# WesleyHsieh0806/TAO-Amodal

Measured on AMD Instinct MI355X. Metric: box-pair IoU+match throughput, higher is better.
Workload: dtype f64

## Files before the change

include/tao_amodal_hip.h:

```cpp
#ifndef TAO_AMODAL_HIP_H
#define TAO_AMODAL_HIP_H

#include <stddef.h>
#include <stdint.h>

#ifdef __cplusplus
extern "C" {
#endif

#define TAOAMD_N_THR 10
#define TAOAMD_N_REC 101
#define TAOAMD_LVIS_RNG 6
#define TAOAMD_TAO_RNG 20

#define TAOAMD_GT_IGNORE 1
#define TAOAMD_GT_OOF 2
#define TAOAMD_GT_ID_HIDDEN 4
#define TAOAMD_DT_IGNORE_UNMATCHED 1
#define TAOAMD_DT_NO_CONSUME 2

#define TAOAMD_OK 0
#define TAOAMD_ERR_HIP 1
#define TAOAMD_ERR_ARG 2
#define TAOAMD_ERR_TOO_LARGE 3
// ... 117 lines not shown
                                  const int64_t *b, int64_t *out, int64_t *n_out);

int taoamd_track_iou_plan_host(int64_t n_cells, const int32_t *cell_dt_off_host,
                               const int32_t *cell_gt_off_host,
                               const int64_t *cell_iou_off_host,
                               const int32_t *trk_meta_host, int64_t *sizes,
                               int32_t *tasks_host, int32_t *task_rows_host,
                               int32_t *task_pairs_host, int64_t *task_out_host);
int taoamd_track_iou_plan_spans_host(int64_t n_cells, const int32_t *cell_dt_off_host,
                                     const int32_t *cell_gt_off_host,
                                     const int64_t *cell_iou_off_host,
                                     const int32_t *trk_meta_host, int64_t *sizes,
                                     int32_t *tasks_host, int32_t *task_rows_host,
                                     int32_t *task_pairs_host, int64_t *task_out_host,
                                     int64_t *zero_out_host);

#define TAOAMD_MAX_GT_PER_CELL 3072
int taoamd_match(int64_t n_cells, const int32_t *cell_dt_off,
                 const int32_t *cell_gt_off, const int64_t *cell_iou_off,
                 int32_t max_gt_per_cell, const double *dt_box,
                 const double *gt_box, const double *iou, int32_t n_rng,
                 const uint32_t *gt_rng, const uint32_t *dt_rng,
                 const uint8_t *gt_flags, const uint8_t *dt_flags,
                 const int32_t *dst, int64_t out_stride, uint64_t *matched,
                 uint64_t *ignored, int32_t *match_gt, double *ious_out,
                 const int32_t *dt_group, const uint32_t *dt_meta,
                 const int32_t *groups, int32_t n_groups, const int32_t *singles,
                 int32_t n_singles, void *stream);

int taoamd_match_compact(int64_t n_cells, const int32_t *cell_dt_off,
                         const int32_t *cell_gt_off, int32_t max_gt_per_cell,
                         const double *dt_box, const double *gt_box, int32_t n_rng,
                         const uint32_t *gt_rng, const uint8_t *gt_flags,
                         const uint8_t *dt_flags, uint64_t *rows, uint32_t *compact,
                         const int32_t *dt_group, const uint32_t *dt_meta,
                         const int32_t *groups, int32_t n_groups, const int32_t *singles,
                         int32_t n_singles, void *stream);
int taoamd_expand_rows(int64_t n_dt, int32_t n_rng, const uint32_t *compact,
                       uint64_t *rows, void *stream);

int taoamd_flat_map(int64_t n, const int64_t *image_id, const int64_t *category_id,
                    const double *bbox, const double *area_in, int64_t n_img,
                    const int64_t *img_ids, int64_t n_cat, const int64_t *cat_ids,
                    int32_t *img, int32_t *cat, double *area, int32_t *img_count,
                    int32_t *img_start, int32_t *img_first, int32_t *status,
                    void *stream);
int taoamd_flat_rank_drop(int64_t n, const int32_t *order, const int32_t *img,
                          const int32_t *img_start, int32_t max_dets,
                          uint8_t *dropped, void *stream);
int taoamd_flat_filter(int64_t n, const int32_t *unit, const int32_t *cat,
                       const double *area, const int64_t *category_id,
                       const uint8_t *dropped, int32_t n_unit, int64_t n_gkeys,
                       const int32_t *gkeys, const int32_t *unit_row,
                       const int64_t *neg_off, const int64_t *neg_val,
                       const int64_t *nel_off, const int64_t *nel_val,
                       int32_t area_flag, int32_t *key, uint8_t *flags,
                       int32_t *n_keep, void *stream);
int taoamd_flat_gather(int64_t n_keep, const int32_t *order, const double *score,
                       const uint8_t *flags, const int32_t *key,
                       const double *bbox, int32_t n_unit, int32_t *dt_row,
                       double *dt_score, uint8_t *dt_flags, int32_t *dt_key,
                       int32_t *dt_cat, double *dt_box, void *stream);
int taoamd_flat_count_bad(int64_t n, const double *bbox, const uint8_t *dropped,
                          int32_t *count, void *stream);
int taoamd_flat_ordscore(int64_t n, const int32_t *img, const int32_t *img_count,
                         const double *score, int32_t max_dets, double *out,
                         void *stream);
int taoamd_flat_ordinal(int64_t n, const int32_t *order, const int32_t *img,
                        const int32_t *img_start, int32_t max_dets,
                        int32_t *ordinal, uint8_t *dropped, void *stream);
int taoamd_flat_merge_cat(int64_t n, const int64_t *category_id, int64_t n_merge,
                          const int64_t *merge_src, const int64_t *merge_dst,
                          int64_t n_cat, const int64_t *cat_ids, int64_t *merged_id,
                          int32_t *cat, void *stream);
int taoamd_flat_split64(int64_t n, const int64_t *key, const int32_t *order,
                        int32_t *lo, int32_t *hi, void *stream);
int taoamd_flat_compose(int64_t n, const int32_t *outer, const int32_t *inner,
                        int32_t *out, void *stream);
int taoamd_flat_gather_cols(int64_t n, const int32_t *idx, const int32_t *src_i32,
                            int32_t *out_i32, const double *src_f64,
                            double *out_f64, const uint8_t *src_u8,
                            uint8_t *out_u8, void *stream);
int taoamd_flat_track_of(int64_t n, const int32_t *order, const int32_t *run_id,
                         const int32_t *run_start, const int64_t *video_id,
                         int32_t *trk, int32_t *status, void *stream);
int taoamd_flat_keys(int64_t n, const int32_t *img, const int32_t *ordinal,
                     const uint8_t *dropped, const int32_t *cat, const double *area,
                     const int32_t *trk, const int32_t *img_rank,
                     const int32_t *visit_rank, const double *img_frame,
                     const int32_t *tl_pos, double M, double *keep_key,
                     double *visit_key, double *frame_key, double *pos_key,
                     int32_t *trk_keep, int32_t *trk_sel, void *stream);
int taoamd_flat_track_kept(int64_t n_runs, const int32_t *run_trk,
                           const int32_t *run_start, int64_t n_sorted,
                           const int32_t *order_k, const double *score,
                           const int64_t *merged_id, double *trk_score,
                           int32_t *trk_first_kept, int32_t *status, void *stream);
int taoamd_flat_track_sel(int64_t n_runs, const int32_t *run_trk,
                          const int32_t *run_start, int64_t n_sorted,
                          const int32_t *order_s, const double *area,
                          const double *visit_key, const int32_t *img,
                          double *sel_area, int32_t *sel_len, int32_t *sel_frames,
                          double *sel_first, void *stream);
int taoamd_flat_track_filter(int64_t n_runs, const int32_t *run_trk,
                             const int32_t *sel_len, const int32_t *trk_first_kept,
                             const int32_t *cat, const int64_t *merged_id,
                             const int64_t *video_id, const int64_t *track_id,
                             int64_t n_vid, const int64_t *vid_ids, int64_t n_gkeys,
                             const int32_t *gkeys, const int32_t *vid_row,
                             const int64_t *neg_off, const int64_t *neg_val,
                             const int64_t *nel_off, const int64_t *nel_val,
                             int32_t *key, uint8_t *flags, int32_t *n_keep,
                             int32_t *status, void *stream);
int taoamd_flat_frames(int64_t n_trk, const int32_t *trk_run,
                       const int32_t *run_start, int64_t n_runs, int64_t n_sorted,
                       const int32_t *order_s, const int32_t *img,
                       const int32_t *tl_pos, const double *bbox,
                       const int32_t *frame_off, int32_t *frame_pos,
                       double *frame_box, void *stream);
int taoamd_flat_scan(int64_t n, const int32_t *count, int32_t *start,
                     int32_t *status2, void *stream);
size_t taoamd_flat_runs_workspace(int64_t n);
int taoamd_flat_runs(int64_t n, const int32_t *sorted_key, int32_t *run_id,
                     int32_t *run_key, int32_t *run_start, int32_t *n_runs,
                     void *workspace, size_t workspace_bytes, void *stream);
int taoamd_flat_runs_by(int64_t n, const int32_t *key, const int32_t *order,
                        int32_t *run_id, int32_t *run_key, int32_t *run_start,
                        int32_t *n_runs, void *workspace, size_t workspace_bytes,
                        void *stream);
int taoamd_flat_runs64_by(int64_t n, const int64_t *key, const int32_t *order,
                          int32_t *run_id, int64_t *run_key, int32_t *run_start,
                          int32_t *n_runs, void *workspace, size_t workspace_bytes,
                          void *stream);
int taoamd_flat_remap(int64_t n, const int32_t *id, const int32_t *map,
                      int32_t *out, void *stream);

int taoamd_match_plan_host(int64_t n_cells, const int32_t *cell_dt_off_host,
                           const int32_t *cell_gt_off_host, int32_t cap_d,
                           int32_t cap_g, int32_t cap_cell_g, int64_t *sizes,
                           int32_t *groups_host, int32_t *singles_host);

size_t taoamd_sort_workspace(int64_t n);
int taoamd_sort_by_cat_score(int64_t n, const int32_t *dt_cat,
                             const double *dt_score, int32_t *order,
                             int32_t *dst, void *workspace,
                             size_t workspace_bytes, void *stream);

#define TAOAMD_SORT_CHUNK (16 * 2816)
int taoamd_sort_plan_host(int32_t n_cat, const int32_t *cat_off_host, int64_t *sizes,
                          int32_t *chunks, int32_t *split_list, int32_t *stile_chunk,
                          int32_t *bucket_chunk);
size_t taoamd_sort_sampled_workspace(int64_t n, int64_t n_buckets, int32_t merge);
int taoamd_sort_sampled_cap_limit(int32_t limit);
int taoamd_sort_sampled(int64_t n, int32_t n_cat, const int32_t *cat_off,
                        const int32_t *tile_off, int32_t n_tiles, int32_t max_segment,
                        const double *dt_score, int32_t n_chunks, const int32_t *chunks,
                        int32_t n_split, const int32_t *split_list, int32_t n_stiles,
                        const int32_t *stile_chunk, int32_t n_buckets,
                        const int32_t *bucket_chunk, int32_t *order, int32_t *dst,
                        void *workspace, size_t workspace_bytes, void *stream);

#define TAOAMD_SEGMENT_TILE 2816
size_t taoamd_sort_segments_workspace(int64_t n);
int taoamd_sort_segments(int64_t n, int32_t n_cat, const int32_t *cat_off,
                         const int32_t *tile_off, int32_t n_tiles,
                         int32_t max_segment, const int32_t *dt_cat,
                         const double *dt_score, int32_t *order, int32_t *dst,
                         void *workspace, size_t workspace_bytes, void *stream);

int taoamd_gather_rows(int64_t n, int32_t n_words, const uint64_t *src_matched,
                       const uint64_t *src_ignored, int64_t src_stride,
                       const int32_t *order, uint64_t *dst_matched,
                       uint64_t *dst_ignored, void *stream);

size_t taoamd_accumulate_workspace(int64_t n_dt, int32_t n_cat, int32_t n_rng);
size_t taoamd_compact_elems(int32_t n_cat, int32_t n_rng);
int taoamd_accumulate_compact(int64_t n_dt, int32_t n_cat, int32_t n_rng,
                              const int32_t *cat_off, const uint64_t *matched,
                              const uint64_t *ignored, const int32_t *num_gt,
                              int32_t k_begin, int32_t k_end, int32_t max_segment,
                              double *val, double *rec, void *workspace,
                              size_t workspace_bytes, void *stream);
int taoamd_finalize(int32_t n_cat, int32_t n_rng, const int32_t *num_gt,
                    const double *val, const double *rec, double *precision,
                    double *recall, void *stream);
int taoamd_accumulate(int64_t n_dt, int32_t n_cat, int32_t n_rng,
                      const int32_t *cat_off, const uint64_t *matched,
                      const uint64_t *ignored,
                      const int32_t *num_gt, int32_t max_segment, double *precision,
                      double *recall, void *workspace, size_t workspace_bytes,
                      void *stream);
int taoamd_accumulate_error(const void *workspace, void *stream, int32_t *flag_host);
int taoamd_accumulate_chunked(int64_t n_dt, int32_t n_cat, int32_t n_rng,
                      const int32_t *cat_off, const uint64_t *matched,
                      const uint64_t *ignored,
                      const int32_t *num_gt, int32_t max_segment, double *precision,
                      double *recall, void *workspace, size_t workspace_bytes,
                      void *stream);
int taoamd_accumulate_compact_chunked(int64_t n_dt, int32_t n_cat, int32_t n_rng,
                              const int32_t *cat_off, const uint64_t *matched,
                              const uint64_t *ignored, const int32_t *num_gt,
                              int32_t k_begin, int32_t k_end, int32_t max_segment,
                              double *val, double *rec, void *workspace,
                              size_t workspace_bytes, void *stream);
int taoamd_accumulate_sweep_mode(int32_t mode);
int taoamd_accumulate_plan_kind(int64_t n_dt, int32_t n_rng, int32_t max_segment);
int taoamd_accumulate_spin_limit(int32_t polls);
int taoamd_accumulate_giveup_counter(uint32_t *device_word);
int taoamd_accumulate_prepare(int64_t n_dt, int32_t n_cat, int32_t n_rng,
                              const int32_t *cat_off, int32_t max_segment,
                              void *workspace, size_t workspace_bytes, void *stream);
int taoamd_accumulate_prepared(int64_t n_dt, int32_t n_cat, int32_t n_rng,
                      const int32_t *cat_off, const uint64_t *matched,
                      const uint64_t *ignored,
                      const int32_t *num_gt, int32_t max_segment, double *precision,
                      double *recall, void *workspace, size_t workspace_bytes,
                      void *stream);
int taoamd_accumulate_by_order(int64_t n_dt, int32_t n_cat, int32_t n_rng,
                               const int32_t *cat_off, const int32_t *order,
                               const uint64_t *matched, const uint64_t *ignored,
                               const int32_t *num_gt, int32_t max_segment,
                               double *precision, double *recall, void *workspace,
                               size_t workspace_bytes, void *stream);
int taoamd_accumulate_by_order_prepared(int64_t n_dt, int32_t n_cat, int32_t n_rng,
                               const int32_t *cat_off, const int32_t *order,
                               const uint64_t *matched, const uint64_t *ignored,
                               const int32_t *num_gt, int32_t max_segment,
                               double *precision, double *recall, void *workspace,
                               size_t workspace_bytes, void *stream);
int taoamd_accumulate_by_order_chunked(int64_t n_dt, int32_t n_cat, int32_t n_rng,
                               const int32_t *cat_off, const int32_t *order,
                               const uint64_t *matched, const uint64_t *ignored,
                               const int32_t *num_gt, int32_t max_segment,
                               double *precision, double *recall, void *workspace,
                               size_t workspace_bytes, void *stream);
int taoamd_accumulate_by_order_compact(int64_t n_dt, int32_t n_cat, int32_t n_rng,
                               const int32_t *cat_off, const int32_t *order,
                               const uint32_t *compact, const uint64_t *rows,
                               const int32_t *num_gt, int32_t max_segment,
                               double *precision, double *recall, void *workspace,
                               size_t workspace_bytes, int32_t prepared, void *stream);

size_t taoamd_score_at_recall_workspace(int64_t n_dt, int32_t n_cat, int32_t n_rng);
int taoamd_score_at_recall(int64_t n_dt, int32_t n_cat, int32_t n_rng,
                           const int32_t *cat_off, const int32_t *order,
                           const uint64_t *matched, const uint64_t *ignored,
                           const double *score, const int32_t *score_order,
                           const int32_t *num_gt, double *scores, void *workspace, size_t workspace_bytes,
                           void *stream);

#define TAOAMD_ERROR_TYPES_TILE 256
#define TAOAMD_ERROR_TYPES_MAX_RNG 8
size_t taoamd_error_types_workspace(int64_t n_dt, int64_t n_gt, int32_t n_rng);
int taoamd_error_types(int64_t n_dt, int64_t n_gt, int32_t n_img, int32_t n_cat,
                       int32_t n_rng, int32_t slot, double bg_thr,
                       const int32_t *dt_cat, const double *dt_box,
                       const uint8_t *dt_flags, const int32_t *dt_gt0,
                       const int32_t *match_gt, int64_t match_stride,
                       const int32_t *gt_cat, const double *gt_box,
                       const uint32_t *gt_rng, const int32_t *img_gt_off,
                       const int32_t *img_gt, const int32_t *img_dt_off,
                       const int32_t *img_dt, int64_t *dt_counts, int64_t *gt_counts,
                       uint8_t *dt_type, void *workspace, size_t workspace_bytes,
                       void *stream);

int taoamd_error_types_links(int64_t n_dt, int64_t n_gt, int32_t n_img, int32_t n_cat,
                             int32_t n_rng, int32_t slot, double bg_thr,
                             const int32_t *dt_cat, const double *dt_box,
                             const uint8_t *dt_flags, const int32_t *dt_gt0,
                             const int32_t *match_gt, int64_t match_stride,
                             const int32_t *gt_cat, const double *gt_box,
                             const uint32_t *gt_rng, const int32_t *img_gt_off,
                             const int32_t *img_gt, const int32_t *img_dt_off,
                             const int32_t *img_dt, int64_t *dt_counts, int64_t *gt_counts,
                             uint8_t *dt_type, int32_t *link_same, int32_t *link_other,
                             uint8_t *held, void *workspace, size_t workspace_bytes,
                             void *stream);

#define TAOAMD_ERROR_IMPACT_FIXES 9
#define TAOAMD_ERROR_IMPACT_CHUNK 256
size_t taoamd_error_impact_workspace(int64_t n_dt, int64_t n_gt, int32_t n_cat, int32_t n_rng);
int taoamd_error_impact(int64_t n_dt, int64_t n_gt, int32_t n_cat, int32_t n_rng,
                        const int32_t *cat_off, const int32_t *order, const double *score,
                        const int32_t *dt_cat, const uint8_t *dt_type,
                        const int32_t *link_same, const int32_t *link_other,
                        const int32_t *gt_cat, const uint32_t *gt_rng, const uint8_t *held,
                        double *precision, int32_t *num_gt, void *workspace,
                        size_t workspace_bytes, void *stream);

size_t taoamd_track_error_impact_workspace(int64_t n_dt, int64_t n_gt, int32_t n_cat,
                                           int32_t n_rng);
int taoamd_track_error_impact(int64_t n_dt, int64_t n_gt, int32_t n_cat, int32_t n_rng,
                              const int32_t *cat_off, const int32_t *order,
                              const double *score, const int32_t *dt_cat,
                              const uint8_t *dt_type, const int32_t *link_same,
                              const int32_t *link_other, const int32_t *gt_cat,
                              const uint32_t *gt_rng, const uint8_t *held, double *precision,
                              int32_t *num_gt, void *workspace, size_t workspace_bytes,
                              void *stream);

#define TAOAMD_CONFUSION_TILE 2048
size_t taoamd_confusion_workspace(int64_t n_dt, int64_t n_gt, int32_t n_cat, int32_t n_rng);
int taoamd_confusion_count(int64_t n_dt, int64_t n_gt, int32_t n_cat, int32_t n_rng,
                           const int32_t *cat_off, const double *score, const int32_t *dt_cat,
                           const uint8_t *dt_type, const int32_t *link_other,
                           const int32_t *gt_cat, const uint8_t *held, int64_t *ent_off,
// ... 232 lines not shown
```

tao_amodal_amd/csrc/sort.hip:

```cpp
#include <algorithm>
#include <cstdlib>
#include <cstring>

#include "common.hpp"
#include "workspace.hpp"

using namespace taoamd;

#define RS_THREADS 256
#define RS_WAVES (RS_THREADS / WAVE)
#define RS_ITEMS 8
#define RS_TILE (RS_THREADS * RS_ITEMS)
#define RS_BINS 256
#define RS_PASSES 12

struct SortBufs {
    uint64_t *key[2];
    int32_t *idx[2];
    const int32_t *cat;
    uint32_t *block_hist;
    uint32_t *digit_total;
    int32_t *skip;
    int32_t *sel;
    int64_t n;
// ... 677 lines not shown
            L.key[i] = kin[src_of(i)];
            L.pos[i] = (uint16_t)i;
        }
    });
    const int32_t out = X.out_base;
#pragma nounroll
    for (int i = threadIdx.x; i < total; i += SEG_THREADS) {
        const int32_t p = out + seg_final_slot(L, i, total, repaired);
        const int32_t d = iin[src_of((int)(L.pos[i] & 0x0fffu))];
        if (a.order) a.order[p] = d;
        if (a.dst) a.dst[d] = p;
    }
}

#define MP_PER 11

template <class KA, class KB>
__device__ __forceinline__ int32_t merge_split(KA A, int32_t na, KB B, int32_t nb, int32_t o)
{
    int32_t lo = max(0, o - nb), hi = min(o, na);
    while (lo < hi) {
        const int32_t mid = (lo + hi) >> 1;
        if (A[mid] <= B[o - mid - 1]) lo = mid + 1; else hi = mid;
    }
    return lo;
}

__global__ __launch_bounds__(256) void seg_mpass_kernel(SegArgs a, int pass, int last,
                                                        int32_t longer_than)
{
    __shared__ uint64_t m_key[SEG_TILE];
    __shared__ int32_t m_idx[SEG_TILE];
    __shared__ int32_t m_split[2];
    static_assert(256 * MP_PER == SEG_TILE, "one workgroup = one tile-sized slice");
    int32_t lo = 0, hi = a.n_cat;
    while (hi - lo > 1) {
        const int32_t mid = (lo + hi) >> 1;
        if (a.tile_off[mid] <= (int32_t)blockIdx.x) lo = mid; else hi = mid;
    }
    const int32_t k = lo;
    const int32_t sb = a.cat_off[k], se = a.cat_off[k + 1];
    if (se - sb <= longer_than) return;
    const int32_t tb = sb + ((int32_t)blockIdx.x - a.tile_off[k]) * SEG_TILE;
    const int32_t len = min(SEG_TILE, se - tb);
    if (len <= 0) return;
    const int s = pass & 1;
    const uint64_t *__restrict__ kin = a.key[s];
    const int32_t *__restrict__ iin = a.idx[s];
    const int64_t L = (int64_t)SEG_TILE << pass;
    const int64_t base = sb + ((tb - sb) / (2 * L)) * (2 * L);
    const int32_t a0 = (int32_t)base, a1 = (int32_t)min(base + L, (int64_t)se);
    const int32_t b1 = (int32_t)min((int64_t)a1 + L, (int64_t)se);
    const int32_t na = a1 - a0, nb = b1 - a1;
    const int32_t o0 = tb - a0;
    auto emit = [&](int32_t p, uint64_t kx, int32_t ix) {
        if (last) {
            if (a.order) a.order[p] = ix;
            if (a.dst) a.dst[ix] = p;
        } else {
            a.key[s ^ 1][p] = kx;
            a.idx[s ^ 1][p] = ix;
        }
    };
    if (nb <= 0) {
        for (int32_t i = threadIdx.x; i < len; i += 256) emit(tb + i, kin[tb + i], iin[tb + i]);
        return;
    }
    if (threadIdx.x == 0) m_split[0] = merge_split(kin + a0, na, kin + a1, nb, o0);
    if (threadIdx.x == 64) m_split[1] = merge_split(kin + a0, na, kin + a1, nb, o0 + len);
    __syncthreads();
    const int32_t i0 = m_split[0], i1 = m_split[1];
    const int32_t j0 = o0 - i0;
    const int32_t pa = i1 - i0, pb = len - pa;
    for (int32_t i = threadIdx.x; i < len; i += 256) {
        const int32_t src = i < pa ? a0 + i0 + i : a1 + j0 + (i - pa);
        m_key[i] = kin[src];
        m_idx[i] = iin[src];
    }
    __syncthreads();
    const int32_t q0 = min(len, (int32_t)threadIdx.x * MP_PER);
    const int32_t q1 = min(len, q0 + MP_PER);
    if (q0 >= q1) return;
    const uint64_t *A = m_key, *B = m_key + pa;
    int32_t ia = merge_split(A, pa, B, pb, q0);
    int32_t ib = q0 - ia;
    for (int32_t q = q0; q < q1; q++) {
        const bool takeA = ib >= pb || (ia < pa && A[ia] <= B[ib]);
        const int32_t from = takeA ? ia : pa + ib;
        emit(tb + q, m_key[from], m_idx[from]);
        ia += takeA ? 1 : 0;
        ib += takeA ? 0 : 1;
    }
}

static void seg_layout(Carve &c, int64_t n, SegArgs &a)
{
    if (n < 1) n = 1;
    key_idx_layout(c, n, a);
    a.bnd = c.take<int32_t>(((size_t)n / SEG_TILE + 2) * SEG_BND_PER_SLOT);
}

extern "C" size_t taoamd_sort_segments_workspace(int64_t n)
{
    SegArgs a;
    return measure([&](Carve &c) { seg_layout(c, n, a); });
}

extern "C" int taoamd_sort_segments(int64_t n, int32_t n_cat,
                                    const int32_t *cat_off,
                                    const int32_t *tile_off, int32_t n_tiles,
                                    int32_t max_segment, const int32_t *dt_cat,
                                    const double *dt_score, int32_t *order,
                                    int32_t *dst, void *workspace,
                                    size_t workspace_bytes, void *stream)
{
    if (n == 0 || n_cat == 0 || n_tiles == 0) return TAOAMD_OK;
    if (n > 0x7fffffff) return TAOAMD_ERR_TOO_LARGE;
    if (!cat_off || !tile_off || !dt_cat || !dt_score || !workspace) return TAOAMD_ERR_ARG;
    Carve c(workspace);
    SegArgs a;
    seg_layout(c, n, a);
    if (!c.fits(workspace, workspace_bytes)) return TAOAMD_ERR_WORKSPACE;
    hipStream_t s = (hipStream_t)stream;
    a.cat_off = cat_off; a.tile_off = tile_off; a.cat = dt_cat; a.score = dt_score;
    a.order = order; a.dst = dst; a.n = n; a.n_cat = n_cat; a.n_tiles = n_tiles;
    TAO_TIMED("seg_tile_kernel", s, seg_tile_kernel<<<(unsigned)n_tiles, SEG_THREADS, 0, s>>>(a));
    if (max_segment > SEG_TILE && max_segment <= (int64_t)SEG_KMERGE_TILES * SEG_TILE) {
        TAO_TIMED("seg_kmerge_kernel", s, seg_kmerge_kernel<<<(unsigned)((n + 255) / 256), 256, 0, s>>>(a));
    } else if (max_segment > SEG_TILE) {
        TAO_TIMED("seg_split_kernel", s, seg_split_kernel<<<(unsigned)n_cat, SEG_THREADS, 0, s>>>(a));
        TAO_TIMED("seg_bucket_kernel", s, seg_bucket_kernel<<<2u * (unsigned)n_tiles, SEG_THREADS, 0, s>>>(a));
        const int32_t longer_than = SEG_SPLIT_TILES * SEG_TILE;
        if (max_segment > longer_than) {
            int passes = 0;
            for (int64_t L = SEG_TILE; L < max_segment; L <<= 1) passes++;
            for (int p = 0; p < passes; p++)
                TAO_TIMED("seg_mpass_kernel", s, seg_mpass_kernel<<<(unsigned)n_tiles, 256, 0, s>>>(a, p, p == passes - 1, longer_than));
        }
    }
    TAO_LAUNCH_CHECK();
    return TAOAMD_OK;
}

#define SS_CAP 1024
#define SS_FAST 512
#define SS_TARGET 352
#define SS_CHUNK_TILES 16
#define SS_FIRST_MERGE_PASS 4
#define SS_OVER 32
#define SS_DIRECT 1024
#define SS_CHUNK (SS_CHUNK_TILES * SEG_TILE)
#define SS_MAXB 128
#define SS_HALF_CHUNK (SS_CHUNK / 2)

struct SsChunk {
    int32_t begin, n;
    int32_t bucket0, n_buckets;
    int32_t stile0;
    int32_t final;
    int32_t cat, pad;
};

struct SsArgs {
    const double *score;
    const SsChunk *chunks;
    const int32_t *split_list, *stile_chunk, *bucket_chunk;
    int32_t *cursor;
    uint64_t *spl_key;
    int32_t *spl_idx;
    uint64_t *slot_key;
    int32_t *slot_idx;
    uint64_t *key_out;
    int32_t *idx_out;
    int32_t *order, *dst;
    int32_t *redo;
    int32_t n_buckets, n_stiles, cap_limit;
};

static int g_ss_cap_limit = SS_CAP;

__host__ __device__ inline int ss_over(int32_t n) { return n > SS_HALF_CHUNK ? SS_OVER / 2 : SS_OVER; }

__device__ __forceinline__ uint32_t ss_mix(uint32_t x)
{
    x ^= x >> 16; x *= 0x7feb352du; x ^= x >> 15; x *= 0x846ca68bu; x ^= x >> 16;
    return x;
}

__device__ __forceinline__ uint64_t ss_shfl_xor64(uint64_t v, int j)
{
    const uint32_t lo = (uint32_t)__shfl_xor((int)(uint32_t)v, j, WAVE);
    const uint32_t hi = (uint32_t)__shfl_xor((int)(uint32_t)(v >> 32), j, WAVE);
    return ((uint64_t)hi << 32) | lo;
}

__device__ __forceinline__ double ss_fmin(double a, double b)
{
    double r;
    asm("v_min_f64 %0, %1, %2" : "=v"(r) : "v"(a), "v"(b));
    return r;
}
__device__ __forceinline__ double ss_fmax(double a, double b)
{
    double r;
    asm("v_max_f64 %0, %1, %2" : "=v"(r) : "v"(a), "v"(b));
    return r;
}
template <int CTRL>
__device__ __forceinline__ double ss_dpp_f64(double v)
{
    const int lo = __builtin_amdgcn_update_dpp(0, __double2loint(v), CTRL, 0xF, 0xF, true);
    const int hi = __builtin_amdgcn_update_dpp(0, __double2hiint(v), CTRL, 0xF, 0xF, true);
    return __hiloint2double(hi, lo);
}
__device__ __forceinline__ double ss_shfl_xor_f64(double v, int m)
{
    switch (m) {
    case 1: return ss_dpp_f64<0xB1>(v);
    case 2: return ss_dpp_f64<0x4E>(v);
    case 3: return ss_dpp_f64<0x1B>(v);
    case 4: return ss_dpp_f64<0x1B>(ss_dpp_f64<0x141>(v));
    case 7: return ss_dpp_f64<0x141>(v);
    case 8: return ss_dpp_f64<0x128>(v);
    case 15: return ss_dpp_f64<0x140>(v);
    default: break;
    }
    const int lo = __shfl_xor(__double2loint(v), m, WAVE);
    const int hi = __shfl_xor(__double2hiint(v), m, WAVE);
    return __hiloint2double(hi, lo);
}

template <int R>
__device__ __forceinline__ void ss_bitonic_packed(double (&p)[R], int lane)
{
    constexpr int LOG_N = 6 + (R == 1 ? 0 : R == 2 ? 1 : R == 4 ? 2 : R == 8 ? 3 : R == 16 ? 4 : 5);
#pragma unroll
    for (int ls = 1; ls <= LOG_N; ls++) {
        const int size = 1 << ls;
        if (size <= R) {
#pragma unroll
            for (int r = 0; r < R; r++) {
                const int r2 = r ^ (size - 1);
                if (r < r2) {
                    const double lo = ss_fmin(p[r], p[r2]), hi = ss_fmax(p[r], p[r2]);
                    p[r] = lo;
                    p[r2] = hi;
                }
            }
        } else {
            const int m = size / R - 1;
            const bool lower = (lane & (size / R / 2)) == 0;
            if (R == 1) {
                const double o = ss_shfl_xor_f64(p[0], m);
                p[0] = ((o < p[0]) == lower) ? o : p[0];
            }
            if (R > 1) {
                constexpr int G = R / 2 < 2 ? 1 : 2;
#pragma unroll
                for (int r0 = 0; r0 < R / 2; r0 += G) {
                    double o1[G], o2[G];
#pragma unroll
                    for (int g = 0; g < G; g++) {
                        o1[g] = ss_shfl_xor_f64(p[R - 1 - (r0 + g)], m);
                        o2[g] = ss_shfl_xor_f64(p[r0 + g], m);
                    }
                    if (lower) {
#pragma unroll
                        for (int g = 0; g < G; g++) {
                            p[r0 + g] = ss_fmin(p[r0 + g], o1[g]);
                            p[R - 1 - (r0 + g)] = ss_fmin(p[R - 1 - (r0 + g)], o2[g]);
                        }
                    } else {
#pragma unroll
                        for (int g = 0; g < G; g++) {
                            p[r0 + g] = ss_fmax(p[r0 + g], o1[g]);
                            p[R - 1 - (r0 + g)] = ss_fmax(p[R - 1 - (r0 + g)], o2[g]);
                        }
                    }
                }
            }
        }
#pragma unroll
        for (int lj = ls - 2; lj >= 0; lj--) {
            const int j = 1 << lj;
            if (j >= R) {
                const int m = j / R;
                const bool lower = (lane & m) == 0;
                constexpr int G = R < 4 ? R : 4;
#pragma unroll
                for (int r0 = 0; r0 < R; r0 += G) {
                    double o[G];
#pragma unroll
                    for (int g = 0; g < G; g++) o[g] = ss_shfl_xor_f64(p[r0 + g], m);
                    if (lower) {
#pragma unroll
                        for (int g = 0; g < G; g++) p[r0 + g] = ss_fmin(p[r0 + g], o[g]);
                    } else {
#pragma unroll
                        for (int g = 0; g < G; g++) p[r0 + g] = ss_fmax(p[r0 + g], o[g]);
                    }
                }
            } else {
#pragma unroll
                for (int r = 0; r < R; r++) {
                    if ((r & j) == 0) {
                        const double lo = ss_fmin(p[r], p[r | j]), hi = ss_fmax(p[r], p[r | j]);
                        p[r] = lo;
                        p[r | j] = hi;
                    }
                }
            }
        }
    }
}

__device__ __forceinline__ uint64_t ss_shfl_up64(uint64_t v)
{
    const uint32_t lo = (uint32_t)__shfl_up((int)(uint32_t)v, 1, WAVE);
    const uint32_t hi = (uint32_t)__shfl_up((int)(uint32_t)(v >> 32), 1, WAVE);
    return ((uint64_t)hi << 32) | lo;
}
__device__ __forceinline__ uint64_t ss_shfl_down64(uint64_t v)
{
    const uint32_t lo = (uint32_t)__shfl_down((int)(uint32_t)v, 1, WAVE);
    const uint32_t hi = (uint32_t)__shfl_down((int)(uint32_t)(v >> 32), 1, WAVE);
    return ((uint64_t)hi << 32) | lo;
}
__device__ __forceinline__ uint64_t ss_wave_min_u64(uint64_t v)
// ... 53 lines not shown
    for (int r = 0; r < R; r++) {
        const int j = (r * 4 + wave) * WAVE + lane;
        p[r] = j < m ? ss_pack(desc_key(sc[r]), 0, 64 - SS_SPLIT_KEY_BITS, rel[r])
                     : __longlong_as_double((long long)SS_PAD);
    }
    ss_bitonic_packed<R>(p, lane);
    int32_t rank[R];
    uint64_t v[R];
#pragma unroll
    for (int r = 0; r < R; r++) {
        v[r] = (uint64_t)__double_as_longlong(p[r]);
        rank[r] = lane * R + r;
    }
#pragma unroll
    for (int k = 0; k < 4; k++) {
        if (wave == k) {
#pragma unroll
            for (int r = 0; r < R; r++) run[lane * R + r] = v[r];
        }
        __syncthreads();
        if (wave != k) {
            constexpr int G = R < 4 ? R : 4;
#pragma unroll
            for (int r0 = 0; r0 < R; r0 += G) {
                int32_t lo[G];
#pragma unroll
                for (int g = 0; g < G; g++) lo[g] = 0;
#pragma unroll
                for (int half = R * WAVE / 2; half > 0; half >>= 1) {
#pragma unroll
                    for (int g = 0; g < G; g++)
                        lo[g] += run[lo[g] + half - 1] < v[r0 + g] ? half : 0;
                }
#pragma unroll
                for (int g = 0; g < G; g++) rank[r0 + g] += lo[g] + (run[lo[g]] < v[r0 + g] ? 1 : 0);
            }
        }
        if (k < 3) __syncthreads();
    }
    int32_t at[R];
    double ks[R];
#pragma unroll
    for (int r = 0; r < R; r++) {
        at[r] = c.begin + (int32_t)(v[r] & ((1u << SS_IDX_BITS) - 1));
        const int q = rank[r] + 1;
        if (v[r] == SS_PAD || q % S != 0 || q / S >= B) at[r] = -1;
    }
#pragma unroll
    for (int r = 0; r < R; r++) ks[r] = a.score[at[r] >= 0 ? at[r] : c.begin];
#pragma unroll
    for (int r = 0; r < R; r++) {
        if (at[r] >= 0) {
            const int q = rank[r] + 1;
            a.spl_key[c.bucket0 + q / S] = desc_key(ks[r]);
            a.spl_idx[c.bucket0 + q / S] = at[r];
        }
    }
}

__global__ __launch_bounds__(256) void ss_split4_kernel(SsArgs a, int32_t n_split)
{
    __shared__ uint64_t run[WAVE * 8];
    const int lane = lane_id();
    const int wave = __builtin_amdgcn_readfirstlane(threadIdx.x >> 6);
    const SsChunk c = a.chunks[a.split_list[blockIdx.x]];
    const int32_t m = ss_over(c.n) * c.n_buckets;
    if (m <= 256) ss_split_chunk4<1>(a, c, lane, wave, run);
    else if (m <= 512) ss_split_chunk4<2>(a, c, lane, wave, run);
    else if (m <= 1024) ss_split_chunk4<4>(a, c, lane, wave, run);
    else ss_split_chunk4<8>(a, c, lane, wave, run);
}

__global__ __launch_bounds__(SEG_THREADS) void ss_scatter_kernel(SsArgs a)
{
    __shared__ uint64_t s_key[SS_MAXB];
    __shared__ int32_t s_idx[SS_MAXB];
    __shared__ int32_t s_cnt[SS_MAXB], s_base[SS_MAXB];
    const uint32_t blk = xcd_block(blockIdx.x, gridDim.x);
    const SsChunk c = a.chunks[a.stile_chunk[blk]];
    const int32_t B = c.n_buckets;
    const int32_t t0 = c.begin + ((int32_t)blk - c.stile0) * SEG_TILE;
    const int32_t t1 = min(t0 + SEG_TILE, c.begin + c.n);
    if (threadIdx.x < SS_MAXB) {
        const int b = threadIdx.x;
        s_cnt[b] = 0;
        const bool real = b >= 1 && b < B;
        s_key[b] = real ? a.spl_key[c.bucket0 + b] : ~0ull;
        s_idx[b] = real ? a.spl_idx[c.bucket0 + b] : INT32_MAX;
    }
    __syncthreads();
    if (threadIdx.x >= 1 && (int)threadIdx.x + 1 < B) {
        const int b = threadIdx.x;
        const bool ok = s_key[b] < s_key[b + 1] ||
                        (s_key[b] == s_key[b + 1] && s_idx[b] < s_idx[b + 1]);
        if (!ok) atomicMax(&a.cursor[c.bucket0], 1 << 30);
    }
    uint64_t kr[SEG_ROUNDS];
    int32_t br[SEG_ROUNDS], rr[SEG_ROUNDS];
#pragma unroll
    for (int r = 0; r < SEG_ROUNDS; r++) {
        const int32_t i = t0 + r * SEG_THREADS + (int32_t)threadIdx.x;
        kr[r] = desc_key(a.score[i < t1 ? i : t0]);
    }
#pragma unroll
    for (int r = 0; r < SEG_ROUNDS; r++) {
        const int32_t i = t0 + r * SEG_THREADS + (int32_t)threadIdx.x;
        br[r] = -1;
        if (i < t1) {
            const uint64_t k = kr[r];
            int lo = 1, hi = B;
            while (lo < hi) {
                const int mid = (lo + hi) >> 1;
                const uint64_t sk = s_key[mid];
                const bool before = sk < k || (sk == k && s_idx[mid] < i);
                if (before) lo = mid + 1; else hi = mid;
            }
            br[r] = lo - 1;
            rr[r] = atomicAdd(&s_cnt[lo - 1], 1);
        }
    }
    __syncthreads();
    if (threadIdx.x < B) {
        const int32_t n = s_cnt[threadIdx.x];
        s_base[threadIdx.x] = n ? atomicAdd(&a.cursor[c.bucket0 + threadIdx.x], n) : 0;
    }
    __syncthreads();
#pragma unroll
    for (int r = 0; r < SEG_ROUNDS; r++) {
        if (br[r] >= 0) {
            const int32_t at = s_base[br[r]] + rr[r];
            if (at < SS_CAP) {
                const int64_t s = (int64_t)(c.bucket0 + br[r]) * SS_CAP + at;
                a.slot_key[s] = kr[r];
                a.slot_idx[s] = t0 + r * SEG_THREADS + (int32_t)threadIdx.x;
            }
        }
    }
}

#define SS_KEY_BITS 35
#define SS_E_BITS 10
typedef int32_t ss_i4 __attribute__((ext_vector_type(4), aligned(4)));
typedef int32_t ss_i2 __attribute__((ext_vector_type(2), aligned(4)));

__device__ __forceinline__ int ss_shift_for(uint64_t range)
{
    const int bits = range ? 64 - __clzll((long long)range) : 0;
    return bits > SS_KEY_BITS ? bits - SS_KEY_BITS : 0;
}

template <int R>
__device__ __forceinline__ bool ss_sort_bucket(const SsArgs &a, const SsChunk &c,
                                               int32_t count, int32_t out0, int lane,
                                               const uint64_t *__restrict__ sk,
                                               const int32_t *__restrict__ si,
                                               uint64_t *__restrict__ full)
{
    static_assert(WAVE * R <= (1 << SS_E_BITS), "slot bits");
    const double pad = __longlong_as_double((long long)SS_PAD);
    uint64_t k[R];
    int32_t x[R];
    uint64_t kmin = ~0ull, kmax = 0;
    if (sk == nullptr) {
#pragma unroll
        for (int r = 0; r < R; r++) {
            const int e = r * WAVE + lane;
            k[r] = desc_key(a.score[c.begin + (e < count ? e : 0)]);
            x[r] = c.begin + e;
        }
    } else {
#pragma unroll
        for (int r = 0; r < R; r++) {
            const int e = r * WAVE + lane;
            k[r] = sk[e < count ? e : 0];
            x[r] = si[e < count ? e : 0];
        }
    }
#pragma unroll
    for (int r = 0; r < R; r++) {
        const int e = r * WAVE + lane;
        if (e < count) {
            kmin = k[r] < kmin ? k[r] : kmin;
            kmax = k[r] > kmax ? k[r] : kmax;
        } else {
            k[r] = ~0ull;
            x[r] = INT32_MAX;
        }
        full[e] = k[r];
    }
    kmin = ss_wave_min_u64(kmin);
    kmax = ss_wave_max_u64(kmax);
    const int shift = ss_shift_for(kmax - kmin);
    double p[R];
#pragma unroll
    for (int r = 0; r < R; r++) {
        const int e = r * WAVE + lane;
        p[r] = e < count
            ? __longlong_as_double((long long)((1ull << 61) |
                  (((k[r] - kmin) >> shift) << (SS_IDX_BITS + SS_E_BITS)) |
                  ((uint64_t)(x[r] - c.begin) << SS_E_BITS) | (uint64_t)e))
            : pad;
    }
    ss_bitonic_packed<R>(p, lane);
    bool bad = false;
#pragma unroll
    for (int r = 0; r < R; r++) {
        const uint64_t bits = (uint64_t)__double_as_longlong(p[r]);
        const bool ok = lane * R + r < count;
        x[r] = c.begin + (int32_t)((bits >> SS_E_BITS) & ((1u << SS_IDX_BITS) - 1));
        k[r] = ok ? full[bits & ((1u << SS_E_BITS) - 1) & (WAVE * R - 1)] : ~0ull;
        if (r > 0) bad |= k[r] < k[r - 1];
    }
    const uint64_t up = ss_shfl_up64(k[R - 1]);
    bad |= lane > 0 && k[0] < up;
    if (__ballot(bad) != 0) return false;
    if (lane * R + R <= count && c.final && a.order) {
        int32_t *o = a.order + out0 + lane * R;
        if (R == 2) *(ss_i2 *)o = ss_i2{x[0], x[1]};
#pragma unroll
        for (int q = 0; q + 4 <= R; q += 4)
            *(ss_i4 *)(o + q) = ss_i4{x[q], x[q + 1], x[q + 2], x[q + 3]};
        if (R == 1) o[0] = x[0];
    }
#pragma unroll
    for (int r = 0; r < R; r++) {
        const int e = lane * R + r;
        if (e < count) {
            const int32_t pp = out0 + e;
            if (c.final) {
                if (a.order && lane * R + R > count) a.order[pp] = x[r];
                if (a.dst) a.dst[x[r]] = pp;
            } else {
                a.key_out[pp] = k[r];
                a.idx_out[pp] = x[r];
            }
        }
    }
    return true;
}

__device__ __forceinline__ void ss_rank_bucket(const SsArgs &a, const SsChunk &c,
                                               int32_t count, int32_t out0, int lane,
                                               const uint64_t *__restrict__ sk,
                                               const int32_t *__restrict__ si)
{
    auto get = [&](int32_t e, uint64_t &k, int32_t &x) {
        if (sk == nullptr) {
            k = desc_key(a.score[c.begin + e]);
            x = c.begin + e;
        } else {
            k = sk[e];
            x = si[e];
        }
    };
    for (int32_t base = 0; base < count; base += WAVE) {
        const int32_t e = base + lane;
        uint64_t k = 0;
        int32_t x = 0, rank = 0;
        if (e < count) get(e, k, x);
        for (int32_t j = 0; j < count; j++) {
            uint64_t kj;
            int32_t xj;
            get(j, kj, xj);
            rank += (kj < k || (kj == k && xj < x)) ? 1 : 0;
        }
        if (e < count) {
            const int32_t pp = out0 + rank;
            if (c.final) {
                if (a.order) a.order[pp] = x;
                if (a.dst) a.dst[x] = pp;
            } else {
                a.key_out[pp] = k;
                a.idx_out[pp] = x;
            }
        }
    }
}

__device__ __forceinline__ bool ss_bucket_geom(const SsArgs &a, int64_t gb, int lane,
                                               SsChunk &c, int32_t &count, int32_t &before,
                                               bool &overflow)
{
    c = a.chunks[a.bucket_chunk[gb]];
    const int32_t b = (int32_t)gb - c.bucket0;
    count = c.n;
    before = 0;
    if (c.n_buckets > 1) {
        const int32_t m0 = lane < c.n_buckets ? a.cursor[c.bucket0 + lane] : 0;
        const int32_t m1 = lane + WAVE < c.n_buckets ? a.cursor[c.bucket0 + WAVE + lane] : 0;
        overflow = __ballot(m0 > a.cap_limit || m1 > a.cap_limit) != 0;
        count = b < WAVE ? __shfl(m0, b, WAVE) : __shfl(m1, b - WAVE, WAVE);
        int32_t pre = (lane < b ? m0 : 0) + (lane + WAVE < b ? m1 : 0);
#pragma unroll
        for (int off = 32; off > 0; off >>= 1) pre += __shfl_xor(pre, off, WAVE);
        before = pre;
    } else {
        overflow = count > a.cap_limit;
    }
    return !overflow;
}

__global__ __launch_bounds__(256) void ss_redo_kernel(SsArgs a)
{
    __shared__ uint64_t s_full[4][WAVE * 16];
    uint64_t *full = s_full[threadIdx.x >> 6];
    const int lane = lane_id();
    const int32_t n = a.redo[-1];
    for (int32_t i = (int32_t)blockIdx.x * 4 + (int32_t)(threadIdx.x >> 6); i < n;
         i += (int32_t)gridDim.x * 4) {
        const int64_t gb = a.redo[i];
        SsChunk c;
        int32_t count, before;
        bool overflow;
        if (!ss_bucket_geom(a, gb, lane, c, count, before, overflow) || count <= 0) continue;
        const uint64_t *sk = nullptr;
        const int32_t *si = nullptr;
        if (c.n_buckets > 1) {
            sk = a.slot_key + gb * SS_CAP;
            si = a.slot_idx + gb * SS_CAP;
        }
        const int32_t out0 = c.begin + before;
        if (count > SS_FAST && ss_sort_bucket<16>(a, c, count, out0, lane, sk, si, full)) continue;
        ss_rank_bucket(a, c, count, out0, lane, sk, si);
    }
}

__global__ __launch_bounds__(256) void ss_sort_kernel(SsArgs a)
{
    __shared__ uint64_t s_full[4][WAVE * 8];
    uint64_t *full = s_full[threadIdx.x >> 6];
    const int lane = lane_id();
    const int64_t gb = (int64_t)xcd_block(blockIdx.x, gridDim.x) * 4 + (threadIdx.x >> 6);
    if (gb >= a.n_buckets) return;
    SsChunk c;
    int32_t count, before;
    bool overflow;
    ss_bucket_geom(a, gb, lane, c, count, before, overflow);
    const int32_t b = (int32_t)gb - c.bucket0;
    if (overflow) {
        const int32_t s0 = (int32_t)((int64_t)c.n * b / c.n_buckets);
        const int32_t s1 = (int32_t)((int64_t)c.n * (b + 1) / c.n_buckets);
        for (int32_t i = s0 + lane; i < s1; i += WAVE) {
            const uint64_t ki = desc_key(a.score[c.begin + i]);
            int32_t rank = 0;
            for (int32_t j = 0; j < c.n; j++) {
                const uint64_t kj = desc_key(a.score[c.begin + j]);
                rank += (kj < ki || (kj == ki && j < i)) ? 1 : 0;
            }
            const int32_t p = c.begin + rank, d = c.begin + i;
            if (c.final) {
                if (a.order) a.order[p] = d;
                if (a.dst) a.dst[d] = p;
            } else {
                a.key_out[p] = ki;
                a.idx_out[p] = d;
            }
        }
        return;
    }
    if (count <= 0) return;
    const int32_t out0 = c.begin + before;
    const uint64_t *sk = nullptr;
    const int32_t *si = nullptr;
    if (c.n_buckets > 1) {
        sk = a.slot_key + gb * SS_CAP;
        si = a.slot_idx + gb * SS_CAP;
    }
    bool done = false;
    if (count <= 64) done = ss_sort_bucket<1>(a, c, count, out0, lane, sk, si, full);
    else if (count <= 128) done = ss_sort_bucket<2>(a, c, count, out0, lane, sk, si, full);
    else if (count <= 256) done = ss_sort_bucket<4>(a, c, count, out0, lane, sk, si, full);
    else if (count <= SS_FAST) done = ss_sort_bucket<8>(a, c, count, out0, lane, sk, si, full);
    if (!done && lane == 0) a.redo[atomicAdd(&a.redo[-1], 1)] = (int32_t)gb;
}

extern "C" int taoamd_sort_plan_host(int32_t n_cat, const int32_t *cat_off_host,
                                     int64_t *sizes, int32_t *chunks,
                                     int32_t *split_list, int32_t *stile_chunk,
                                     int32_t *bucket_chunk)
{
    if (n_cat < 0 || !cat_off_host || !sizes) return TAOAMD_ERR_ARG;
    const bool fill = chunks != nullptr;
    if (fill && (!split_list || !stile_chunk || !bucket_chunk)) return TAOAMD_ERR_ARG;
    int64_t nc = 0, ns = 0, nt = 0, nb = 0, merge = 0;
    for (int32_t k = 0; k < n_cat; k++) {
        const int64_t sb = cat_off_host[k], len = cat_off_host[k + 1] - sb;
        if (len < 0) return TAOAMD_ERR_ARG;
        if (len > SS_CHUNK) merge = 1;
        for (int64_t o = 0; o < len; o += SS_CHUNK) {
            const int32_t n = (int32_t)std::min<int64_t>(SS_CHUNK, len - o);
            const int32_t B = n <= SS_DIRECT ? 1 : (n + SS_TARGET - 1) / SS_TARGET;
            const int32_t tiles = B > 1 ? (n + SEG_TILE - 1) / SEG_TILE : 0;
            if (fill) {
                SsChunk c;
                c.begin = (int32_t)(sb + o); c.n = n; c.bucket0 = (int32_t)nb;
                c.n_buckets = B; c.stile0 = (int32_t)nt; c.final = len <= SS_CHUNK;
                c.cat = k; c.pad = 0;
                memcpy(chunks + 8 * nc, &c, sizeof c);
                if (B > 1) split_list[ns] = (int32_t)nc;
                for (int32_t t = 0; t < tiles; t++) stile_chunk[nt + t] = (int32_t)nc;
                for (int32_t b = 0; b < B; b++) bucket_chunk[nb + b] = (int32_t)nc;
            }
            nc++;
            ns += B > 1;
            nt += tiles;
            nb += B;
        }
    }
    if (nb >= INT32_MAX / 2) return TAOAMD_ERR_TOO_LARGE;
    sizes[0] = nc; sizes[1] = ns; sizes[2] = nt; sizes[3] = nb; sizes[4] = merge;
    return TAOAMD_OK;
}

static size_t ss_layout(Carve &c, int64_t n, int64_t n_buckets, int merge, SsArgs &a, SegArgs &m)
{
    if (n < 1) n = 1;
    if (n_buckets < 1) n_buckets = 1;
    const size_t nb = (size_t)n_buckets;
    const size_t cursor_ints = align256((nb + 64) * 4) / 4;
    a.cursor = c.take<int32_t>(cursor_ints + nb);
    a.redo = Carve::at(a.cursor, cursor_ints);
    a.spl_key = c.take<uint64_t>(nb);
    a.spl_idx = c.take<int32_t>(nb);
    a.slot_key = c.take<uint64_t>(nb * SS_CAP);
    a.slot_idx = c.take<int32_t>(nb * SS_CAP);
    m.key[0] = m.key[1] = nullptr; m.idx[0] = m.idx[1] = nullptr; m.bnd = nullptr;
    if (merge) key_idx_layout(c, n, m);
    return cursor_ints;
}

extern "C" size_t taoamd_sort_sampled_workspace(int64_t n, int64_t n_buckets, int32_t merge)
{
    SsArgs a;
    SegArgs m;
    return measure([&](Carve &c) { ss_layout(c, n, n_buckets, merge, a, m); });
}

extern "C" int taoamd_sort_sampled_cap_limit(int32_t limit)
{
    g_ss_cap_limit = limit > 0 && limit < SS_CAP ? limit : SS_CAP;
    return TAOAMD_OK;
}

extern "C" int taoamd_sort_sampled(int64_t n, int32_t n_cat, const int32_t *cat_off,
                                   const int32_t *tile_off, int32_t n_tiles,
                                   int32_t max_segment, const double *dt_score,
                                   int32_t n_chunks, const int32_t *chunks,
                                   int32_t n_split, const int32_t *split_list,
                                   int32_t n_stiles, const int32_t *stile_chunk,
                                   int32_t n_buckets, const int32_t *bucket_chunk,
                                   int32_t *order, int32_t *dst, void *workspace,
                                   size_t workspace_bytes, void *stream)
{
    if (n == 0 || n_cat == 0 || n_chunks == 0) return TAOAMD_OK;
    if (n > 0x7fffffff) return TAOAMD_ERR_TOO_LARGE;
    if (!cat_off || !dt_score || !chunks || !bucket_chunk || !workspace ||
        (n_split > 0 && (!split_list || !stile_chunk)))
        return TAOAMD_ERR_ARG;
    const int merge = max_segment > SS_CHUNK;
    if (merge && (!tile_off || n_tiles <= 0)) return TAOAMD_ERR_ARG;
    Carve c(workspace);
    SsArgs a;
    SegArgs m;
    const size_t cursor_ints = ss_layout(c, n, n_buckets, merge, a, m);
    if (!c.fits(workspace, workspace_bytes)) return TAOAMD_ERR_WORKSPACE;
    hipStream_t s = (hipStream_t)stream;
    a.score = dt_score; a.chunks = (const SsChunk *)chunks; a.split_list = split_list;
    a.stile_chunk = stile_chunk; a.bucket_chunk = bucket_chunk;
    a.order = order; a.dst = dst; a.n_buckets = n_buckets; a.n_stiles = n_stiles;
    a.cap_limit = g_ss_cap_limit;
    m.cat_off = cat_off; m.tile_off = tile_off; m.cat = nullptr; m.score = dt_score;
    m.order = order; m.dst = dst; m.n = n; m.n_cat = n_cat; m.n_tiles = n_tiles;
    a.key_out = m.key[SS_FIRST_MERGE_PASS & 1];
    a.idx_out = m.idx[SS_FIRST_MERGE_PASS & 1];
    TAO_HIP(hipMemsetAsync(a.cursor, 0, cursor_ints * 4, s));
    if (n_split > 0) {
        TAO_TIMED("ss_split_kernel", s, ss_split4_kernel<<<(unsigned)n_split, 256, 0, s>>>(a, n_split));
        TAO_TIMED("ss_scatter_kernel", s, ss_scatter_kernel<<<(unsigned)n_stiles, SEG_THREADS, 0, s>>>(a));
    }
    TAO_TIMED("ss_sort_kernel", s, ss_sort_kernel<<<(unsigned)((n_buckets + 3) / 4), 256, 0, s>>>(a));
    TAO_TIMED("ss_redo_kernel", s, ss_redo_kernel<<<(unsigned)std::min<int64_t>(1024, (n_buckets + 3) / 4), 256, 0, s>>>(a));
    if (merge) {
        int passes = 0;
        for (int64_t L = SEG_TILE; L < max_segment; L <<= 1) passes++;
        for (int p = SS_FIRST_MERGE_PASS; p < passes; p++)
            TAO_TIMED("seg_mpass_kernel", s, seg_mpass_kernel<<<(unsigned)n_tiles, 256, 0, s>>>(m, p, p == passes - 1, SS_CHUNK));
    }
    TAO_LAUNCH_CHECK();
    return TAOAMD_OK;
}
```

Before: 49120.

## Sort oversized buckets inline via two-run sort plus merge, drop redo kernel

```diff
diff --git a/include/tao_amodal_hip.h b/include/tao_amodal_hip.h
--- a/include/tao_amodal_hip.h
+++ b/include/tao_amodal_hip.h
@@ -293,6 +293,8 @@
                           int32_t *bucket_chunk);
 size_t taoamd_sort_sampled_workspace(int64_t n, int64_t n_buckets, int32_t merge);
 int taoamd_sort_sampled_cap_limit(int32_t limit);
+int taoamd_sort_sampled_paths(void *workspace, int64_t n, int64_t n_buckets, int32_t merge,
+                              void *stream, int32_t *out);
 int taoamd_sort_sampled(int64_t n, int32_t n_cat, const int32_t *cat_off,
                         const int32_t *tile_off, int32_t n_tiles, int32_t max_segment,
                         const double *dt_score, int32_t n_chunks, const int32_t *chunks,
diff --git a/tao_amodal_amd/csrc/sort.hip b/tao_amodal_amd/csrc/sort.hip
--- a/tao_amodal_amd/csrc/sort.hip
+++ b/tao_amodal_amd/csrc/sort.hip
@@ -853,6 +853,7 @@
 #define SS_CHUNK (SS_CHUNK_TILES * SEG_TILE)
 #define SS_MAXB 128
 #define SS_HALF_CHUNK (SS_CHUNK / 2)
+#define SS_MERGE_G 3
 
 struct SsChunk {
     int32_t begin, n;
@@ -874,7 +875,7 @@
     uint64_t *key_out;
     int32_t *idx_out;
     int32_t *order, *dst;
-    int32_t *redo;
+    int32_t *paths;
     int32_t n_buckets, n_stiles, cap_limit;
 };
 
@@ -1234,8 +1235,7 @@
 template <int R>
 __device__ __forceinline__ bool ss_sort_bucket(const SsArgs &a, const SsChunk &c,
                                                int32_t count, int32_t out0, int lane,
-                                               const uint64_t *__restrict__ sk,
-                                               const int32_t *__restrict__ si,
+                                               const uint64_t *sk, const int32_t *si,
                                                uint64_t *__restrict__ full)
 {
     static_assert(WAVE * R <= (1 << SS_E_BITS), "slot bits");
@@ -1321,30 +1321,51 @@
     return true;
 }
 
+__device__ __forceinline__ uint64_t ss_peek(const uint64_t *p)
+{
+    return __hip_atomic_load(p, __ATOMIC_RELAXED, __HIP_MEMORY_SCOPE_AGENT);
+}
+__device__ __forceinline__ int32_t ss_peek(const int32_t *p)
+{
+    return __hip_atomic_load(p, __ATOMIC_RELAXED, __HIP_MEMORY_SCOPE_AGENT);
+}
+__device__ __forceinline__ void ss_stores_done()
+{
+    asm volatile("s_waitcnt vmcnt(0)" ::: "memory");
+}
+
 __device__ __forceinline__ void ss_rank_bucket(const SsArgs &a, const SsChunk &c,
                                                int32_t count, int32_t out0, int lane,
-                                               const uint64_t *__restrict__ sk,
-                                               const int32_t *__restrict__ si)
+                                               const uint64_t *sk, const int32_t *si)
 {
     auto get = [&](int32_t e, uint64_t &k, int32_t &x) {
         if (sk == nullptr) {
             k = desc_key(a.score[c.begin + e]);
             x = c.begin + e;
         } else {
-            k = sk[e];
-            x = si[e];
+            k = ss_peek(sk + e);
+            x = ss_peek(si + e);
         }
     };
+    asm volatile("" : "+v"(lane));
     for (int32_t base = 0; base < count; base += WAVE) {
         const int32_t e = base + lane;
         uint64_t k = 0;
         int32_t x = 0, rank = 0;
         if (e < count) get(e, k, x);
-        for (int32_t j = 0; j < count; j++) {
-            uint64_t kj;
-            int32_t xj;
-            get(j, kj, xj);
-            rank += (kj < k || (kj == k && xj < x)) ? 1 : 0;
+        for (int32_t jb = 0; jb < count; jb += WAVE) {
+            uint64_t kl = 0;
+            int32_t xl = 0;
+            if (jb + lane < count) get(jb + lane, kl, xl);
+            const int32_t nj = min(WAVE, count - jb);
+#pragma nounroll
+            for (int32_t t = 0; t < nj; t++) {
+                const uint64_t kj =
+                    ((uint64_t)(uint32_t)__builtin_amdgcn_readlane((int)(kl >> 32), t) << 32) |
+                    (uint32_t)__builtin_amdgcn_readlane((int)kl, t);
+                const int32_t xj = __builtin_amdgcn_readlane(xl, t);
+                rank += (kj < k || (kj == k && xj < x)) ? 1 : 0;
+            }
         }
         if (e < count) {
             const int32_t pp = out0 + rank;
@@ -1382,32 +1403,142 @@
     return !overflow;
 }
 
-__global__ __launch_bounds__(256) void ss_redo_kernel(SsArgs a)
-{
-    __shared__ uint64_t s_full[4][WAVE * 16];
-    uint64_t *full = s_full[threadIdx.x >> 6];
-    const int lane = lane_id();
-    const int32_t n = a.redo[-1];
-    for (int32_t i = (int32_t)blockIdx.x * 4 + (int32_t)(threadIdx.x >> 6); i < n;
-         i += (int32_t)gridDim.x * 4) {
-        const int64_t gb = a.redo[i];
-        SsChunk c;
-        int32_t count, before;
-        bool overflow;
-        if (!ss_bucket_geom(a, gb, lane, c, count, before, overflow) || count <= 0) continue;
-        const uint64_t *sk = nullptr;
-        const int32_t *si = nullptr;
-        if (c.n_buckets > 1) {
-            sk = a.slot_key + gb * SS_CAP;
-            si = a.slot_idx + gb * SS_CAP;
-        }
-        const int32_t out0 = c.begin + before;
-        if (count > SS_FAST && ss_sort_bucket<16>(a, c, count, out0, lane, sk, si, full)) continue;
-        ss_rank_bucket(a, c, count, out0, lane, sk, si);
-    }
-}
-
-__global__ __launch_bounds__(256) void ss_sort_kernel(SsArgs a)
+template <int G>
+__device__ __forceinline__ void ss_merge_runs(const SsArgs &a, const SsChunk &c,
+                                              int32_t count, int32_t out0, int lane,
+                                              const uint64_t *pk, const int32_t *pi,
+                                              uint64_t *full)
+{
+    asm volatile("" : "+v"(lane));
+#pragma nounroll
+    for (int run = 0; run < 2; run++) {
+        const int32_t n_mine = run ? count - SS_FAST : SS_FAST, n_other = count - n_mine;
+        const uint64_t *mk = pk + (run ? SS_FAST : 0), *ok = pk + (run ? 0 : SS_FAST);
+        const int32_t *mi = pi + (run ? SS_FAST : 0), *oi = pi + (run ? 0 : SS_FAST);
+#pragma nounroll
+        for (int32_t e0 = 0; e0 < n_mine; e0 += G * WAVE) {
+#pragma nounroll
+            for (int q = 0; q < SS_FAST; q += 4 * WAVE) {
+                uint64_t t[4];
+#pragma unroll
+                for (int r = 0; r < 4; r++) {
+                    const uint32_t e = (uint32_t)(q + r * WAVE + lane);
+                    t[r] = ss_peek(ok + (e < (uint32_t)n_other ? e : 0u));
+                }
+#pragma unroll
+                for (int r = 0; r < 4; r++) full[q + r * WAVE + lane] = t[r];
+            }
+            uint64_t k[G];
+            uint32_t lo[G], hi[G];
+#pragma unroll
+            for (int g = 0; g < G; g++) {
+                const uint32_t e = (uint32_t)(e0 + g * WAVE + lane);
+                k[g] = ss_peek(mk + (e < (uint32_t)n_mine ? e : 0u));
+                lo[g] = hi[g] = 0;
+            }
+#pragma nounroll
+            for (int it = 0; it < 10; it++) {
+                const uint32_t step = it < 9 ? (uint32_t)(SS_FAST / 2) >> it : 1u;
+                uint64_t kl[G], kh[G];
+#pragma unroll
+                for (int g = 0; g < G; g++) {
+                    kl[g] = full[lo[g] + step - 1];
+                    kh[g] = full[hi[g] + step - 1];
+                }
+#pragma unroll
+                for (int g = 0; g < G; g++) {
+                    const uint32_t jl = lo[g] + step - 1, jh = hi[g] + step - 1;
+                    lo[g] += jl < (uint32_t)n_other && kl[g] < k[g] ? step : 0u;
+                    hi[g] += jh < (uint32_t)n_other && kh[g] <= k[g] ? step : 0u;
+                }
+            }
+            int32_t x[G];
+            bool ties = false;
+#pragma unroll
+            for (int g = 0; g < G; g++) {
+                const uint32_t e = (uint32_t)(e0 + g * WAVE + lane);
+                x[g] = ss_peek(mi + (e < (uint32_t)n_mine ? e : 0u));
+                ties |= hi[g] > lo[g];
+            }
+            if (__ballot(ties) != 0) {
+#pragma nounroll
+                for (int q = 0; q < SS_FAST; q += 4 * WAVE) {
+                    int32_t t[4];
+#pragma unroll
+                    for (int r = 0; r < 4; r++) {
+                        const uint32_t e = (uint32_t)(q + r * WAVE + lane);
+                        t[r] = ss_peek(oi + (e < (uint32_t)n_other ? e : 0u));
+                    }
+#pragma unroll
+                    for (int r = 0; r < 4; r++)
+                        full[q + r * WAVE + lane] = (uint64_t)(uint32_t)t[r];
+                }
+#pragma nounroll
+                for (int it = 0; it < 10; it++) {
+                    const uint32_t step = it < 9 ? (uint32_t)(SS_FAST / 2) >> it : 1u;
+                    int32_t xl[G];
+#pragma unroll
+                    for (int g = 0; g < G; g++) {
+                        const uint32_t j = lo[g] + step - 1;
+                        xl[g] = (int32_t)(uint32_t)full[j < SS_FAST ? j : 0u];
+                    }
+#pragma unroll
+                    for (int g = 0; g < G; g++) {
+                        const uint32_t j = lo[g] + step - 1;
+                        lo[g] += j < hi[g] && xl[g] < x[g] ? step : 0u;
+                    }
+                }
+            }
+#pragma unroll
+            for (int g = 0; g < G; g++) {
+                const int32_t e = e0 + g * WAVE + lane;
+                if (e < n_mine) {
+                    const int32_t pp = out0 + e + (int32_t)lo[g];
+                    if (c.final) {
+                        if (a.order) a.order[pp] = x[g];
+                        if (a.dst) a.dst[x[g]] = pp;
+                    } else {
+                        a.key_out[pp] = ss_peek(mk + e);
+                        a.idx_out[pp] = x[g];
+                    }
+                }
+            }
+        }
+    }
+}
+
+__device__ __forceinline__ bool ss_sort_upto_fast(const SsArgs &a, const SsChunk &c,
+                                                  int32_t m, int32_t out0, int lane,
+                                                  const uint64_t *sk, const int32_t *si,
+                                                  uint64_t *full)
+{
+    if (m <= 64) return ss_sort_bucket<1>(a, c, m, out0, lane, sk, si, full);
+    if (m <= 128) return ss_sort_bucket<2>(a, c, m, out0, lane, sk, si, full);
+    if (m <= 256) return ss_sort_bucket<4>(a, c, m, out0, lane, sk, si, full);
+    return ss_sort_bucket<8>(a, c, m, out0, lane, sk, si, full);
+}
+
+__device__ __forceinline__ bool ss_sort_run(const SsArgs &a, const SsChunk &c, int32_t base,
+                                            int32_t m, int lane, const uint64_t *sk,
+                                            const int32_t *si, uint64_t *full,
+                                            uint64_t *pk, int32_t *pi)
+{
+    asm volatile("" : "+v"(lane));
+    SsArgs ar = a;
+    SsChunk cr = c;
+    ar.key_out = pk;
+    ar.idx_out = pi;
+    cr.final = 0;
+    if (sk == nullptr) {
+        cr.begin += base;
+    } else {
+        sk += base;
+        si += base;
+    }
+    return ss_sort_upto_fast(ar, cr, m, base, lane, sk, si, full);
+}
+
+__global__ __launch_bounds__(256, 8) void ss_sort_kernel(SsArgs a)
 {
     __shared__ uint64_t s_full[4][WAVE * 8];
     uint64_t *full = s_full[threadIdx.x >> 6];
@@ -1448,12 +1579,21 @@
         sk = a.slot_key + gb * SS_CAP;
         si = a.slot_idx + gb * SS_CAP;
     }
-    bool done = false;
-    if (count <= 64) done = ss_sort_bucket<1>(a, c, count, out0, lane, sk, si, full);
-    else if (count <= 128) done = ss_sort_bucket<2>(a, c, count, out0, lane, sk, si, full);
-    else if (count <= 256) done = ss_sort_bucket<4>(a, c, count, out0, lane, sk, si, full);
-    else if (count <= SS_FAST) done = ss_sort_bucket<8>(a, c, count, out0, lane, sk, si, full);
-    if (!done && lane == 0) a.redo[atomicAdd(&a.redo[-1], 1)] = (int32_t)gb;
+    const bool big = count > SS_FAST;
+    bool done;
+    if (!big) {
+        done = ss_sort_upto_fast(a, c, count, out0, lane, sk, si, full);
+        if (done) return;
+    } else {
+        uint64_t *pk = a.slot_key + gb * SS_CAP;
+        int32_t *pi = a.slot_idx + gb * SS_CAP;
+        done = ss_sort_run(a, c, 0, SS_FAST, lane, sk, si, full, pk, pi) &&
+               ss_sort_run(a, c, SS_FAST, count - SS_FAST, lane, sk, si, full, pk, pi);
+        ss_stores_done();
+        if (done) ss_merge_runs<SS_MERGE_G>(a, c, count, out0, lane, pk, pi, full);
+    }
+    if (!done) ss_rank_bucket(a, c, count, out0, lane, sk, si);
+    if (lane == 0) atomicAdd(&a.paths[done ? 0 : 1], 1);
 }
 
 extern "C" int taoamd_sort_plan_host(int32_t n_cat, const int32_t *cat_off_host,
@@ -1500,8 +1640,8 @@
     if (n_buckets < 1) n_buckets = 1;
     const size_t nb = (size_t)n_buckets;
     const size_t cursor_ints = align256((nb + 64) * 4) / 4;
-    a.cursor = c.take<int32_t>(cursor_ints + nb);
-    a.redo = Carve::at(a.cursor, cursor_ints);
+    a.cursor = c.take<int32_t>(cursor_ints);
+    a.paths = Carve::at(a.cursor, nb);
     a.spl_key = c.take<uint64_t>(nb);
     a.spl_idx = c.take<int32_t>(nb);
     a.slot_key = c.take<uint64_t>(nb * SS_CAP);
@@ -1521,6 +1661,20 @@
 extern "C" int taoamd_sort_sampled_cap_limit(int32_t limit)
 {
     g_ss_cap_limit = limit > 0 && limit < SS_CAP ? limit : SS_CAP;
+    return TAOAMD_OK;
+}
+
+extern "C" int taoamd_sort_sampled_paths(void *workspace, int64_t n, int64_t n_buckets,
+                                         int32_t merge, void *stream, int32_t *out)
+{
+    if (!workspace || !out) return TAOAMD_ERR_ARG;
+    Carve c(workspace);
+    SsArgs a;
+    SegArgs m;
+    ss_layout(c, n, n_buckets, merge, a, m);
+    hipStream_t s = (hipStream_t)stream;
+    TAO_HIP(hipMemcpyAsync(out, a.paths, 2 * sizeof(int32_t), hipMemcpyDeviceToHost, s));
+    TAO_HIP(hipStreamSynchronize(s));
     return TAOAMD_OK;
 }
 
@@ -1561,7 +1715,6 @@
         TAO_TIMED("ss_scatter_kernel", s, ss_scatter_kernel<<<(unsigned)n_stiles, SEG_THREADS, 0, s>>>(a));
     }
     TAO_TIMED("ss_sort_kernel", s, ss_sort_kernel<<<(unsigned)((n_buckets + 3) / 4), 256, 0, s>>>(a));
-    TAO_TIMED("ss_redo_kernel", s, ss_redo_kernel<<<(unsigned)std::min<int64_t>(1024, (n_buckets + 3) / 4), 256, 0, s>>>(a));
     if (merge) {
         int passes = 0;
         for (int64_t L = SEG_TILE; L < max_segment; L <<= 1) passes++;
```

After: 48890. No clear change (-0.5%).
